# kan-bayashi/espnet

Hardware: AMD Instinct MI355X
Metric: frames/sec, 12L Conformer hybrid CTC/attention training step (B=32 T=1000 d=256 per GPU) (higher is better)
Workload: dtype f32; 1 GPU; BASELINE configs[1]: 12L Conformer enc d=256 h=4 ff=2048 k=31 macaron+cnn rel_pos, 6L Transformer dec, V=5000, fbank B=32 T=1000 L=100, mtlalpha 0.3, lsm 0.1; global_batch=32, frames=1000, parallelism=dp1, optimizer=adam+noam, clip 5.0, launch=hipGraph, wgrad_side_stream=False, optimizer_steps_done=114

## Files before the change

### espnet_amd/csrc/attn_f32.hip

```cpp
#include "common.h"

namespace {

constexpr int ATT_DK = 64;
constexpr int ATT_MAXK = 512;
constexpr int PLD = 68;

struct AttnF32Args {
  const float* qu; const float* qv; const float* k; const float* v; const float* pos;
  const unsigned char* mask;
  float* P; float* ctx;
  long ldq, ldqv, ldk, ldv, ldpos, ldc, ldp, mb, mi;
  int B, H, T1, T2, nqb;
  float scale;
  float* Pd; float drop_p; const unsigned long long* drop_step; unsigned long long drop_salt;
  const int* tshift;
};

__device__ __forceinline__ float xmax16_32(float v) {
  v = fmaxf(v, __shfl_xor(v, 16));
  return fmaxf(v, __shfl_xor(v, 32));
}
__device__ __forceinline__ float xsum16_32(float v) {
  v += __shfl_xor(v, 16);
  return v + __shfl_xor(v, 32);
}

__device__ __forceinline__ void load_frag(const float* row, int fq, float4 (&f)[4]) {
#pragma unroll
  for (int j = 0; j < 4; ++j) f[j] = *reinterpret_cast<const float4*>(row + 16 * j + 4 * fq);
}
__device__ __forceinline__ f32x4 dot_tile(const float4 (&x)[4], const float4 (&y)[4], f32x4 c) {
#pragma unroll
  for (int j = 0; j < 4; ++j) {
    c = __builtin_amdgcn_mfma_f32_16x16x4f32(x[j].x, y[j].x, c, 0, 0, 0);
    c = __builtin_amdgcn_mfma_f32_16x16x4f32(x[j].y, y[j].y, c, 0, 0, 0);
    c = __builtin_amdgcn_mfma_f32_16x16x4f32(x[j].z, y[j].z, c, 0, 0, 0);
    c = __builtin_amdgcn_mfma_f32_16x16x4f32(x[j].w, y[j].w, c, 0, 0, 0);
  }
  return c;
}

template <int NKT>
__device__ __forceinline__ void panel_load(const float* src, long ld, int rows, int t, float4 (&r)[NKT]) {
#pragma unroll
  for (int q = 0; q < NKT; ++q) {
    const int c = t + 256 * q, row = c >> 4, c4 = c & 15;
    r[q] = *reinterpret_cast<const float4*>(src + (long)min(row, rows - 1) * ld + c4 * 4);
    if (row >= rows) r[q] = make_float4(0.f, 0.f, 0.f, 0.f);
  }
}
template <int NKT>
__device__ __forceinline__ void panel_store(const float4 (&r)[NKT], float* dst, int t) {
#pragma unroll
  for (int q = 0; q < NKT; ++q) {
    const int c = t + 256 * q, row = c >> 4, c4 = c & 15;
    *reinterpret_cast<float4*>(&dst[row * PLD + c4 * 4]) = r[q];
  }
}

template <int NKT>
__device__ __forceinline__ void panel_product(const float* panel, const f32x4 (&G)[NKT], int fr, int fq, f32x4 (&C)[4]) {
#pragma unroll
  for (int kt = 0; kt < NKT; ++kt)
#pragma unroll
    for (int r = 0; r < 4; ++r) {
      const float* row = &panel[(kt * 16 + 4 * fq + r) * PLD + fr];
#pragma unroll
      for (int dt = 0; dt < 4; ++dt) C[dt] = __builtin_amdgcn_mfma_f32_16x16x4f32(row[dt * 16], G[kt][r], C[dt], 0, 0, 0);
    }
}

template <int NKT, bool ACC>
__device__ __forceinline__ void score_tiles(const float* keys, long ldk, int T2, const float* qs, long ldq, int nq,
                                            float* X, int XLD, int wave, int fr, int fq) {
  constexpr int TPW = NKT / 4;
  float4 qf[4][4];
#pragma unroll
  for (int qt = 0; qt < 4; ++qt) load_frag(qs + (long)min(qt * 16 + fr, nq - 1) * ldq, fq, qf[qt]);
#pragma unroll
  for (int u = 0; u < TPW; ++u) {
    const int kt = wave * TPW + u;
    float4 kf[4];
    load_frag(keys + (long)min(kt * 16 + fr, T2 - 1) * ldk, fq, kf);
#pragma unroll
    for (int qt = 0; qt < 4; ++qt) {
      f32x4 c = (f32x4){0.f, 0.f, 0.f, 0.f};
      float4* xp = reinterpret_cast<float4*>(&X[(qt * 16 + fr) * XLD + kt * 16 + 4 * fq]);
      if (ACC) {
        const float4 o = *xp;
        c = (f32x4){o.x, o.y, o.z, o.w};
      }
      c = dot_tile(kf, qf[qt], c);
      *xp = make_float4(c[0], c[1], c[2], c[3]);
    }
  }
}

template <bool REL, int NKT>
__global__ __launch_bounds__(256, NKT > 16 ? 1 : 2) void attn_f32_fwd_kernel(const AttnF32Args a) {
  extern __shared__ __attribute__((aligned(16))) char smem_raw[];
  constexpr int XLD = NKT * 16 + 4;
  constexpr int TPW = NKT / 4;
  const int t = threadIdx.x, lane = t & 63, wave = t >> 6;
  const int fr = lane & 15, fq = lane >> 4;
  const int xcd = blockIdx.x & 7, jb = blockIdx.x >> 3;
  const int z = (jb / a.nqb) * 8 + xcd;
  const bool live = z < a.B * a.H;
  const int zz = live ? z : 0;
  const int h = zz / a.B, b = zz % a.B;
  const int T1 = a.T1, T2 = a.T2;
  const int r0w = min((jb % a.nqb) * 64, T1 - 1);
  const int nq = T1 - r0w;
  const int r0 = r0w + wave * 16;
  const bool active = live && r0 < T1;
  const int qi = min(r0 + fr, T1 - 1);

  float* X = reinterpret_cast<float*>(smem_raw);
  const int Ts = (REL && a.tshift) ? min(max(a.tshift[0], 1), T2) : T2;
  if (REL) {
    if (Ts < T2) {
      for (int e = t; e < 64 * XLD; e += 256) X[e] = 0.f;
      __syncthreads();
    }
    float4 qf[4][4];
    const float* qs = a.qv + ((long)b * T1 + r0w) * a.ldqv + h * ATT_DK;
#pragma unroll
    for (int qt = 0; qt < 4; ++qt) load_frag(qs + (long)min(qt * 16 + fr, nq - 1) * a.ldqv, fq, qf[qt]);
    if (t < 64 && r0w + t + 1 < T2) X[t * XLD + r0w + t + 1] = 0.f;
#pragma unroll
    for (int u = 0; u < TPW; ++u) {
      const int mt = wave * TPW + u;
      float4 pf[4];
      load_frag(a.pos + (long)min(mt * 16 + fr, T2 - 1) * a.ldpos + h * ATT_DK, fq, pf);
#pragma unroll
      for (int qt = 0; qt < 4; ++qt) {
        const f32x4 c = dot_tile(pf, qf[qt], (f32x4){0.f, 0.f, 0.f, 0.f});
        const int ql = qt * 16 + fr, i = r0w + ql;
        const int lim = Ts - 1 - i;
#pragma unroll
        for (int r = 0; r < 4; ++r) {
          const int m = mt * 16 + 4 * fq + r;
          const int row = m >= lim ? ql : ql - 1, j = m >= lim ? m - lim : m + i + 1;
          if (m < Ts && i < Ts && ql < nq && row >= 0) X[row * XLD + j] = c[r];
        }
      }
    }
    const int i64 = r0w + 64;
    if (live && i64 < Ts) {
      const float4* qr = reinterpret_cast<const float4*>(a.qv + ((long)b * T1 + i64) * a.ldqv + h * ATT_DK);
      for (int m = t; m <= Ts - 2 - i64; m += 256) {
        const float4* pr = reinterpret_cast<const float4*>(a.pos + (long)m * a.ldpos + h * ATT_DK);
        float s = 0.f;
#pragma unroll
        for (int j = 0; j < 16; ++j) {
          const float4 x = qr[j], y = pr[j];
          s += x.x * y.x + x.y * y.y + x.z * y.z + x.w * y.w;
        }
        X[63 * XLD + m + i64 + 1] = s;
      }
    }
    __syncthreads();
  }
  score_tiles<NKT, REL>(a.k + (long)b * T2 * a.ldk + h * ATT_DK, a.ldk, T2, a.qu + ((long)b * T1 + r0w) * a.ldq + h * ATT_DK,
                        a.ldq, nq, X, XLD, wave, fr, fq);
  float4 vreg[NKT];
  panel_load<NKT>(a.v + (long)b * T2 * a.ldv + h * ATT_DK, a.ldv, live ? T2 : 1, t, vreg);
  __syncthreads();
  f32x4 S[NKT];
  if (active) {
    unsigned mk[NKT];
    if (a.mask) {
      const unsigned char* mr = a.mask + (long)b * a.mb + (long)qi * a.mi;
#pragma unroll
      for (int kt = 0; kt < NKT; ++kt) {
        const int j0 = kt * 16 + fq * 4;
        const unsigned m0 = mr[min(j0, T2 - 1)], m1 = mr[min(j0 + 1, T2 - 1)], m2 = mr[min(j0 + 2, T2 - 1)],
                       m3 = mr[min(j0 + 3, T2 - 1)];
        mk[kt] = m0 | (m1 << 8) | (m2 << 16) | (m3 << 24);
      }
    } else {
#pragma unroll
      for (int kt = 0; kt < NKT; ++kt) mk[kt] = 0x01010101u;
    }
    const float* xrow = &X[(wave * 16 + fr) * XLD + 4 * fq];
    float mx = -INFINITY;
#pragma unroll
    for (int kt = 0; kt < NKT; ++kt) {
      const int j0 = kt * 16 + fq * 4;
      const float4 xv = *reinterpret_cast<const float4*>(xrow + kt * 16);
      const float xs[4] = {xv.x, xv.y, xv.z, xv.w};
#pragma unroll
      for (int r = 0; r < 4; ++r) {
        float x = xs[r] * a.scale;
        if (j0 + r >= T2 || ((mk[kt] >> (8 * r)) & 0xffu) == 0u) x = -INFINITY;
        S[kt][r] = x;
        mx = fmaxf(mx, x);
      }
    }
    mx = xmax16_32(mx);
    const bool dead = mx == -INFINITY;
    float sum = 0.f;
#pragma unroll
    for (int kt = 0; kt < NKT; ++kt)
#pragma unroll
      for (int r = 0; r < 4; ++r) {
        const float e = dead ? 0.f : __expf(S[kt][r] - mx);
        S[kt][r] = e;
        sum += e;
      }
    sum = xsum16_32(sum);
    const float inv = dead ? 0.f : 1.f / sum;
    const bool qok = r0 + fr < T1;
    const long pro = ((long)zz * T1 + qi) * a.ldp;
    float* prow = a.P + pro;
#pragma unroll
    for (int kt = 0; kt < NKT; ++kt) {
      S[kt] *= inv;
      const int j0 = kt * 16 + fq * 4;
      if (qok && j0 < a.ldp)
        *reinterpret_cast<float4*>(prow + j0) = make_float4(S[kt][0], S[kt][1], S[kt][2], S[kt][3]);
    }
    if (a.drop_p > 0.f) {
      const unsigned seed = eamd_drop_seed(a.drop_step, a.drop_salt), thr = eamd_drop_thr16(a.drop_p);
      const float dinv = eamd_drop_inv(thr);
#pragma unroll
      for (int kt = 0; kt < NKT; ++kt) {
        const int j0 = kt * 16 + fq * 4;
        bool kp[4];
        eamd_drop_keep4(seed, (unsigned long long)(pro + min(j0, (int)a.ldp - 4)), thr, kp);
#pragma unroll
        for (int r = 0; r < 4; ++r) S[kt][r] = kp[r] ? S[kt][r] * dinv : 0.f;
        if (qok && j0 < a.ldp)
          *reinterpret_cast<float4*>(a.Pd + pro + j0) = make_float4(S[kt][0], S[kt][1], S[kt][2], S[kt][3]);
      }
    }
  } else {
#pragma unroll
    for (int kt = 0; kt < NKT; ++kt) S[kt] = (f32x4){0.f, 0.f, 0.f, 0.f};
  }
  __syncthreads();
  float* Vs = reinterpret_cast<float*>(smem_raw);
  panel_store<NKT>(vreg, Vs, t);
  __syncthreads();
  if (!active) return;
  f32x4 C[4];
#pragma unroll
  for (int dt = 0; dt < 4; ++dt) C[dt] = (f32x4){0.f, 0.f, 0.f, 0.f};
  panel_product<NKT>(Vs, S, fr, fq, C);
  if (r0 + fr < T1) {
    float* crow = a.ctx + ((long)b * T1 + r0 + fr) * a.ldc + h * ATT_DK;
#pragma unroll
    for (int dt = 0; dt < 4; ++dt)
      *reinterpret_cast<float4*>(crow + dt * 16 + fq * 4) = make_float4(C[dt][0], C[dt][1], C[dt][2], C[dt][3]);
  }
}

struct AttnF32BwdArgs {
  const float* dctx; const float* k; const float* v; const float* P;
  float* dS; float* dbd; float* dq;
  long ldd, ldk, ldv, ldp, ldo;
  int B, H, T1, T2, nqb;
  float scale;
  float drop_p; const unsigned long long* drop_step; unsigned long long drop_salt;
  const int* tshift;
};

template <int NKT>
__global__ __launch_bounds__(256, NKT > 16 ? 1 : 2) void attn_f32_bwd_q_kernel(const AttnF32BwdArgs a) {
  extern __shared__ __attribute__((aligned(16))) char smem_raw[];
  constexpr int XLD = NKT * 16 + 4;
  const int t = threadIdx.x, lane = t & 63, wave = t >> 6;
  const int fr = lane & 15, fq = lane >> 4;
  const int xcd = blockIdx.x & 7, jb = blockIdx.x >> 3;
  const int z = (jb / a.nqb) * 8 + xcd;
  const bool live = z < a.B * a.H;
  const int zz = live ? z : 0;
  const int h = zz / a.B, b = zz % a.B;
  const int T1 = a.T1, T2 = a.T2;
  const int Ts = (a.dbd && a.tshift) ? min(max(a.tshift[0], 1), T2) : T2;
  const int r0w = min((jb % a.nqb) * 64, T1 - 1);
  const int nq = T1 - r0w;
  const int r0 = r0w + wave * 16;
  const bool active = live && r0 < T1;
  const int qi = min(r0 + fr, T1 - 1);
  const bool qok = r0 + fr < T1;

  float* X = reinterpret_cast<float*>(smem_raw);
  score_tiles<NKT, false>(a.v + (long)b * T2 * a.ldv + h * ATT_DK, a.ldv, T2,
                          a.dctx + ((long)b * T1 + r0w) * a.ldd + h * ATT_DK, a.ldd, nq, X, XLD, wave, fr, fq);
  const float* prow = a.P + ((long)zz * T1 + qi) * a.ldp;
  float4 Pr[NKT];
#pragma unroll
  for (int kt = 0; kt < NKT; ++kt) {
    const int j0 = kt * 16 + fq * 4;
    Pr[kt] = *reinterpret_cast<const float4*>(prow + min(j0, (int)a.ldp - 4));
    if (j0 >= (int)a.ldp) Pr[kt] = make_float4(0.f, 0.f, 0.f, 0.f);
  }
  __syncthreads();
  f32x4 S[NKT];
  if (active) {
    const float* xrow = &X[(wave * 16 + fr) * XLD + 4 * fq];
    const bool drop = a.drop_p > 0.f;
    const unsigned seed = drop ? eamd_drop_seed(a.drop_step, a.drop_salt) : 0u, thr = eamd_drop_thr16(a.drop_p);
    const float dinv = eamd_drop_inv(thr);
    const long pro = ((long)zz * T1 + qi) * a.ldp;
    float s = 0.f;
#pragma unroll
    for (int kt = 0; kt < NKT; ++kt) {
      const int j0 = kt * 16 + fq * 4;
      const float4 xv = *reinterpret_cast<const float4*>(xrow + kt * 16);
      S[kt] = (f32x4){xv.x, xv.y, xv.z, xv.w};
      if (drop) {
        bool kp[4];
        eamd_drop_keep4(seed, (unsigned long long)(pro + min(j0, (int)a.ldp - 4)), thr, kp);
#pragma unroll
        for (int r = 0; r < 4; ++r) S[kt][r] = kp[r] ? S[kt][r] * dinv : 0.f;
      }
      const float pr[4] = {Pr[kt].x, Pr[kt].y, Pr[kt].z, Pr[kt].w};
#pragma unroll
      for (int r = 0; r < 4; ++r) if (j0 + r < T2) s += pr[r] * S[kt][r];
    }
    s = xsum16_32(s);
    const long zo = (long)zz * T1 * a.ldp;
    float* srow = a.dS + zo + (long)qi * a.ldp;
    const int i = r0 + fr;
#pragma unroll
    for (int kt = 0; kt < NKT; ++kt) {
      const int j0 = kt * 16 + fq * 4;
      const float pr[4] = {Pr[kt].x, Pr[kt].y, Pr[kt].z, Pr[kt].w};
#pragma unroll
      for (int r = 0; r < 4; ++r) {
        const int j = j0 + r;
        const float g = j < T2 ? pr[r] * (S[kt][r] - s) * a.scale : 0.f;
        S[kt][r] = g;
        if (a.dbd && qok) {
          if (j < Ts && i < Ts) {
            const int R = j <= i ? i : i + 1, c = j <= i ? Ts + j - i : j - i - 1;
            if (c != 0) a.dbd[zo + (long)R * a.ldp + (c - 1)] = g;
          } else if (j < (int)a.ldp) {
            a.dbd[zo + (long)i * a.ldp + j] = 0.f;
          }
        }
      }
      if (qok && j0 < (int)a.ldp) *reinterpret_cast<float4*>(srow + j0) = make_float4(S[kt][0], S[kt][1], S[kt][2], S[kt][3]);
    }
    if (a.dbd && r0 == 0)
      for (int f = 1 + lane; f < Ts; f += 64) a.dbd[zo + (f - 1)] = 0.f;
  } else {
#pragma unroll
    for (int kt = 0; kt < NKT; ++kt) S[kt] = (f32x4){0.f, 0.f, 0.f, 0.f};
  }
  float4 kreg[NKT];
  panel_load<NKT>(a.k + (long)b * T2 * a.ldk + h * ATT_DK, a.ldk, live ? T2 : 1, t, kreg);
  __syncthreads();
  float* Ks = reinterpret_cast<float*>(smem_raw);
  panel_store<NKT>(kreg, Ks, t);
  __syncthreads();
  if (!active) return;
  f32x4 C[4];
#pragma unroll
  for (int dt = 0; dt < 4; ++dt) C[dt] = (f32x4){0.f, 0.f, 0.f, 0.f};
  panel_product<NKT>(Ks, S, fr, fq, C);
  if (qok) {
    float* orow = a.dq + ((long)b * T1 + r0 + fr) * a.ldo + h * ATT_DK;
#pragma unroll
    for (int dt = 0; dt < 4; ++dt)
      *reinterpret_cast<float4*>(orow + dt * 16 + fq * 4) = make_float4(C[dt][0], C[dt][1], C[dt][2], C[dt][3]);
  }
}

constexpr int ATT_LONG_MAXK = 4096;

typedef unsigned short bfbits;
__device__ __forceinline__ float bf2f_(unsigned short b) { return __uint_as_float((unsigned)b << 16); }
__device__ __forceinline__ float4 ld4(const float* p) { return *reinterpret_cast<const float4*>(p); }
__device__ __forceinline__ float4 ld4(const bfbits* p) {
  const uint2 u = *reinterpret_cast<const uint2*>(p);
  return make_float4(bf2f_(u.x & 0xffffu), bf2f_(u.x >> 16), bf2f_(u.y & 0xffffu), bf2f_(u.y >> 16));
}
__device__ __forceinline__ void st4(float* p, float4 v) { *reinterpret_cast<float4*>(p) = v; }
__device__ __forceinline__ void st4(bfbits* p, float4 v) {
  uint2 u;
  u.x = (unsigned)eamd_f2bf(v.x) | ((unsigned)eamd_f2bf(v.y) << 16);
  u.y = (unsigned)eamd_f2bf(v.z) | ((unsigned)eamd_f2bf(v.w) << 16);
  *reinterpret_cast<uint2*>(p) = u;
}
__device__ __forceinline__ void st1(float* p, float v) { *p = v; }
__device__ __forceinline__ void st1(bfbits* p, float v) { *p = eamd_f2bf(v); }
__device__ __forceinline__ float rnd(const float*, float v) { return v; }
__device__ __forceinline__ float rnd(const bfbits*, float v) { return bf2f_(eamd_f2bf(v)); }
template <typename T>
__device__ __forceinline__ void load_frag_t(const T* row, int fq, float4 (&f)[4]) {
#pragma unroll
  for (int j = 0; j < 4; ++j) f[j] = ld4(row + 16 * j + 4 * fq);
}

template <typename T>
__device__ __forceinline__ void tile_load(const T* src, long ld, int key0, int T2, int lane, float4 (&r)[4]) {
#pragma unroll
  for (int q = 0; q < 4; ++q) {
    const int c = lane + 64 * q, row = c >> 4, c4 = c & 15;
    r[q] = ld4(src + (long)min(key0 + row, T2 - 1) * ld + c4 * 4);
    if (key0 + row >= T2) r[q] = make_float4(0.f, 0.f, 0.f, 0.f);
  }
}
__device__ __forceinline__ void tile_store(const float4 (&r)[4], float* dst, int lane) {
#pragma unroll
  for (int q = 0; q < 4; ++q) {
    const int c = lane + 64 * q, row = c >> 4, c4 = c & 15;
    *reinterpret_cast<float4*>(&dst[row * PLD + c4 * 4]) = r[q];
  }
}
__device__ __forceinline__ void tile_product(const float* tile, const f32x4& G, int fr, int fq, f32x4 (&C)[4]) {
#pragma unroll
  for (int r = 0; r < 4; ++r) {
    const float* row = &tile[(4 * fq + r) * PLD + fr];
#pragma unroll
    for (int dt = 0; dt < 4; ++dt) C[dt] = __builtin_amdgcn_mfma_f32_16x16x4f32(row[dt * 16], G[r], C[dt], 0, 0, 0);
  }
}
template <int NW, typename T>
__device__ __forceinline__ void reduce_store_ct(const f32x4 (&C)[4], float* scr, int wave, int fr, int fq, int t, T* out,
                                                long ld, int nq) {
#pragma unroll
  for (int dt = 0; dt < 4; ++dt)
#pragma unroll
    for (int r = 0; r < 4; ++r) scr[(wave * 64 + dt * 16 + fq * 4 + r) * 17 + fr] = C[dt][r];
  __syncthreads();
  const int q = t >> 4, c4 = (t & 15) * 4;
  if (q < nq) {
    float o[4];
#pragma unroll
    for (int e = 0; e < 4; ++e) {
      float v = 0.f;
#pragma unroll
      for (int w = 0; w < NW; ++w) v += scr[(w * 64 + c4 + e) * 17 + q];
      o[e] = v;
    }
    st4(out + (long)q * ld + c4, make_float4(o[0], o[1], o[2], o[3]));
  }
}

template <typename T, bool REL, int LQ, int NW>
__global__ __launch_bounds__(64 * NW) void attn_fwd_long_kernel(const AttnF32Args a, const int nkt) {
  constexpr int QT = LQ >= 16 ? LQ / 16 : 1;
  constexpr int NT = 64 * NW;
  const T* const a_qu = reinterpret_cast<const T*>(a.qu); const T* const a_qv = reinterpret_cast<const T*>(a.qv);
  const T* const a_k = reinterpret_cast<const T*>(a.k); const T* const a_v = reinterpret_cast<const T*>(a.v);
  const T* const a_pos = reinterpret_cast<const T*>(a.pos);
  T* const a_P = reinterpret_cast<T*>(a.P); T* const a_Pd = reinterpret_cast<T*>(a.Pd); T* const a_ctx = reinterpret_cast<T*>(a.ctx);
  extern __shared__ __attribute__((aligned(16))) char smem_raw[];
  const int XLD = nkt * 16 + 4;
  const int t = threadIdx.x, lane = t & 63, wave = t >> 6;
  const int fr = lane & 15, fq = lane >> 4;
  const int xcd = blockIdx.x & 7, jb = blockIdx.x >> 3;
  const int z = (jb / a.nqb) * 8 + xcd;
  const bool live = z < a.B * a.H;
  const int zz = live ? z : 0;
  const int h = zz / a.B, b = zz % a.B;
  const int T1 = a.T1, T2 = a.T2;
  const int r0w = min((jb % a.nqb) * LQ, T1 - 1);
  const int nq = min(LQ, T1 - r0w);
  int rowx[QT], qrow[QT], qi[QT];
  bool qok[QT];
#pragma unroll
  for (int qt = 0; qt < QT; ++qt) {
    rowx[qt] = min(fr + 16 * qt, LQ - 1);
    qrow[qt] = r0w + min(fr + 16 * qt, nq - 1);
    qi[qt] = min(r0w + rowx[qt], T1 - 1);
    qok[qt] = live && fr + 16 * qt < nq;
  }
  float* X = reinterpret_cast<float*>(smem_raw);
  float* Tw = X + LQ * XLD + wave * 16 * PLD;
  float* red = X + LQ * XLD + NW * 16 * PLD;
  const int Ts = (REL && a.tshift) ? min(max(a.tshift[0], 1), T2) : T2;
  if (REL) {
    if (Ts < T2) {
      for (int e = t; e < LQ * XLD; e += NT) X[e] = 0.f;
      __syncthreads();
    }
    float4 qf[QT][4];
#pragma unroll
    for (int qt = 0; qt < QT; ++qt) load_frag_t(a_qv + ((long)b * T1 + qrow[qt]) * a.ldqv + h * ATT_DK, fq, qf[qt]);
    if (t < LQ && r0w + t + 1 < T2) X[t * XLD + r0w + t + 1] = 0.f;
    float4 pf[4], pfn[4];
    if (wave < nkt) load_frag_t(a_pos + (long)min(wave * 16 + fr, T2 - 1) * a.ldpos + h * ATT_DK, fq, pf);
    for (int mt = wave; mt < nkt; mt += NW) {
      if (mt + NW < nkt) load_frag_t(a_pos + (long)min((mt + NW) * 16 + fr, T2 - 1) * a.ldpos + h * ATT_DK, fq, pfn);
#pragma unroll
      for (int qt = 0; qt < QT; ++qt) {
        const f32x4 c = dot_tile(pf, qf[qt], (f32x4){0.f, 0.f, 0.f, 0.f});
        const int lr = fr + 16 * qt;
        const int i = r0w + lr, lim = Ts - 1 - i;
#pragma unroll
        for (int r = 0; r < 4; ++r) {
          const int m = mt * 16 + 4 * fq + r;
          const int row = m >= lim ? lr : lr - 1, j = m >= lim ? m - lim : m + i + 1;
          if (m < Ts && i < Ts && lr < nq && row >= 0) X[row * XLD + j] = c[r];
        }
      }
#pragma unroll
// ... 172 lines not shown
    qok[qt] = live && fr + 16 * qt < nq;
  }
  float* X = reinterpret_cast<float*>(smem_raw);
  float* Tw = X + LQ * XLD + wave * 16 * PLD;
  float* red = X + LQ * XLD + NW * 16 * PLD;
  const bool drop = a.drop_p > 0.f;
  const unsigned seed = drop ? eamd_drop_seed(a.drop_step, a.drop_salt) : 0u, thr = eamd_drop_thr16(a.drop_p);
  const float dinv = eamd_drop_inv(thr);
  float s[QT];
  {
    float4 df[QT][4];
#pragma unroll
    for (int qt = 0; qt < QT; ++qt) {
      s[qt] = 0.f;
      load_frag_t(a_dctx + ((long)b * T1 + qrow[qt]) * a.ldd + h * ATT_DK, fq, df[qt]);
    }
    const T* vs = a_v + (long)b * T2 * a.ldv + h * ATT_DK;
    float4 vf[4], vfn[4];
    if (wave < nkt) load_frag_t(vs + (long)min(wave * 16 + fr, T2 - 1) * a.ldv, fq, vf);
    for (int kt = wave; kt < nkt; kt += NW) {
      if (kt + NW < nkt) load_frag_t(vs + (long)min((kt + NW) * 16 + fr, T2 - 1) * a.ldv, fq, vfn);
      const int j0 = kt * 16 + fq * 4;
#pragma unroll
      for (int qt = 0; qt < QT; ++qt) {
        f32x4 c = dot_tile(vf, df[qt], (f32x4){0.f, 0.f, 0.f, 0.f});
        float4 pr = ld4(a_P + pro[qt] + min(j0, (int)a.ldp - 4));
        if (j0 >= (int)a.ldp) pr = make_float4(0.f, 0.f, 0.f, 0.f);
        if (drop) {
          bool kp[4];
          eamd_drop_keep4(seed, (unsigned long long)(pro[qt] + min(j0, (int)a.ldp - 4)), thr, kp);
#pragma unroll
          for (int r = 0; r < 4; ++r) c[r] = kp[r] ? c[r] * dinv : 0.f;
        }
        const float p4[4] = {pr.x, pr.y, pr.z, pr.w};
#pragma unroll
        for (int r = 0; r < 4; ++r) if (j0 + r < T2) s[qt] += p4[r] * c[r];
        *reinterpret_cast<float4*>(&X[rowx[qt] * XLD + kt * 16 + 4 * fq]) = make_float4(c[0], c[1], c[2], c[3]);
      }
#pragma unroll
      for (int j = 0; j < 4; ++j) vf[j] = vfn[j];
    }
  }
#pragma unroll
  for (int qt = 0; qt < QT; ++qt) {
    s[qt] = xsum16_32(s[qt]);
    if (fq == 0) red[wave * LQ + rowx[qt]] = s[qt];
  }
  __syncthreads();
#pragma unroll
  for (int qt = 0; qt < QT; ++qt) {
    const int rx = rowx[qt];
    float s_ = 0.f;
#pragma unroll
    for (int w_ = 0; w_ < NW; w_ += 2) s_ += red[w_ * LQ + rx] + red[(w_ + 1) * LQ + rx];
    s[qt] = s_;
  }
  const T* ks = a_k + (long)b * T2 * a.ldk + h * ATT_DK;
  f32x4 C[QT][4];
#pragma unroll
  for (int qt = 0; qt < QT; ++qt)
#pragma unroll
    for (int dt = 0; dt < 4; ++dt) C[qt][dt] = (f32x4){0.f, 0.f, 0.f, 0.f};
  float4 kreg[4];
  if (wave < nkt) tile_load(ks, a.ldk, wave * 16, live ? T2 : 1, lane, kreg);
  for (int kt = wave; kt < nkt; kt += NW) {
    tile_store(kreg, Tw, lane);
    if (kt + NW < nkt) tile_load(ks, a.ldk, (kt + NW) * 16, live ? T2 : 1, lane, kreg);
    const int j0 = kt * 16 + fq * 4;
#pragma unroll
    for (int qt = 0; qt < QT; ++qt) {
      const int i = r0w + fr + 16 * qt;
      float4 pr = ld4(a_P + pro[qt] + min(j0, (int)a.ldp - 4));
      if (j0 >= (int)a.ldp) pr = make_float4(0.f, 0.f, 0.f, 0.f);
      const float4 dp = *reinterpret_cast<const float4*>(&X[rowx[qt] * XLD + kt * 16 + 4 * fq]);
      const float p4[4] = {pr.x, pr.y, pr.z, pr.w}, d4[4] = {dp.x, dp.y, dp.z, dp.w};
      f32x4 G;
#pragma unroll
      for (int r = 0; r < 4; ++r) {
        const int j = j0 + r;
        const float g = j < T2 ? p4[r] * (d4[r] - s[qt]) * a.scale : 0.f;
        G[r] = g;
        if (a.dbd && qok[qt]) {
          if (j < Ts && i < Ts) {
            const int R = j <= i ? i : i + 1, c = j <= i ? Ts + j - i : j - i - 1;
            if (c != 0) st1(a_dbd + zo + (long)R * a.ldp + (c - 1), g);
          } else if (j < (int)a.ldp) {
            st1(a_dbd + zo + (long)i * a.ldp + j, 0.f);
          }
        }
      }
      if (qok[qt] && j0 < (int)a.ldp) st4(a_dS + pro[qt] + j0, make_float4(G[0], G[1], G[2], G[3]));
#pragma unroll
      for (int r = 0; r < 4; ++r) G[r] = rnd(a_dS, G[r]);
      tile_product(Tw, G, fr, fq, C[qt]);
    }
  }
  if (a.dbd && live && r0w == 0)
    for (int f = 1 + t; f < Ts; f += NT) st1(a_dbd + zo + (f - 1), 0.f);
  __syncthreads();
#pragma unroll
  for (int qt = 0; qt < QT; ++qt) {
    if (qt > 0) __syncthreads();
    const int nqt = live ? max(0, min(16, nq - 16 * qt)) : 0;
    const long orow = ((long)b * T1 + r0w + 16 * qt) * a.ldo + h * ATT_DK;
    if (dq_bf16)
      reduce_store_ct<NW>(C[qt], X, wave, fr, fq, t, reinterpret_cast<bfbits*>(a.dq) + orow, a.ldo, nqt);
    else
      reduce_store_ct<NW>(C[qt], X, wave, fr, fq, t, a.dq + orow, a.ldo, nqt);
  }
}

template <typename T, bool REL, int LQ, int NW>
int launch_fwd_long_q(AttnF32Args a, hipStream_t stream) {
  const int nkt = (a.T2 + 15) / 16;
  const size_t smem = ((size_t)LQ * (nkt * 16 + 4) + NW * 16 * PLD + 2 * NW * LQ) * sizeof(float);
  if (smem > 160 * 1024 || smem < (size_t)NW * 64 * 17 * sizeof(float)) return EAMD_EUNSUPPORTED;
  static const hipError_t attr_err = hipFuncSetAttribute(reinterpret_cast<const void*>(&attn_fwd_long_kernel<T, REL, LQ, NW>),
                                                         hipFuncAttributeMaxDynamicSharedMemorySize, 160 * 1024);
  if (attr_err != hipSuccess) return (int)attr_err;
  a.nqb = (a.T1 + LQ - 1) / LQ;
  const int nz = (a.B * a.H + 7) / 8 * 8;
  if ((long)a.nqb * nz >= (1L << 31)) return EAMD_EUNSUPPORTED;
  hipLaunchKernelGGL((attn_fwd_long_kernel<T, REL, LQ, NW>), dim3((unsigned)(a.nqb * nz)), dim3(64 * NW), smem, stream, a, nkt);
  EAMD_LAUNCH_CHECK();
  return EAMD_OK;
}
struct LongGeom { int lq, nw; };
inline LongGeom long_geom(int T1, int T2) {
  const int nkt = (T2 + 15) / 16;
  auto bytes = [&](int lq, int nw) { return ((size_t)lq * (nkt * 16 + 4) + nw * 16 * PLD + 2 * nw * lq) * sizeof(float); };
  LongGeom g{16, 4};
  if (bytes(16, 4) > 160 * 1024) g = LongGeom{8, 4};
  if (bytes(g.lq, 4) > 80 * 1024) g.nw = bytes(g.lq, 8) <= 160 * 1024 ? 8 : bytes(g.lq, 6) <= 160 * 1024 ? 6 : 4;
  (void)T1;
  return g;
}
template <typename T, bool REL>
int launch_fwd_long(AttnF32Args a, hipStream_t stream) {
  const LongGeom g = long_geom(a.T1, a.T2);
  if (g.lq == 16) return g.nw == 8 ? launch_fwd_long_q<T, REL, 16, 8>(a, stream) : g.nw == 6 ? launch_fwd_long_q<T, REL, 16, 6>(a, stream)
                                                                                               : launch_fwd_long_q<T, REL, 16, 4>(a, stream);
  return g.nw == 8 ? launch_fwd_long_q<T, REL, 8, 8>(a, stream) : g.nw == 6 ? launch_fwd_long_q<T, REL, 8, 6>(a, stream)
                                                                              : launch_fwd_long_q<T, REL, 8, 4>(a, stream);
}

template <typename T, int LQ, int NW>
int launch_bwd_long_q(AttnF32BwdArgs a, int dq_bf16, hipStream_t stream) {
  const int nkt = (a.T2 + 15) / 16;
  const size_t smem = ((size_t)LQ * (nkt * 16 + 4) + NW * 16 * PLD + 2 * NW * LQ) * sizeof(float);
  if (smem > 160 * 1024 || smem < (size_t)NW * 64 * 17 * sizeof(float)) return EAMD_EUNSUPPORTED;
  static const hipError_t attr_err = hipFuncSetAttribute(reinterpret_cast<const void*>(&attn_bwd_q_long_kernel<T, LQ, NW>),
                                                         hipFuncAttributeMaxDynamicSharedMemorySize, 160 * 1024);
  if (attr_err != hipSuccess) return (int)attr_err;
  a.nqb = (a.T1 + LQ - 1) / LQ;
  const int nz = (a.B * a.H + 7) / 8 * 8;
  if ((long)a.nqb * nz >= (1L << 31)) return EAMD_EUNSUPPORTED;
  hipLaunchKernelGGL((attn_bwd_q_long_kernel<T, LQ, NW>), dim3((unsigned)(a.nqb * nz)), dim3(64 * NW), smem, stream, a, nkt, dq_bf16);
  EAMD_LAUNCH_CHECK();
  return EAMD_OK;
}
template <typename T>
int launch_bwd_long(AttnF32BwdArgs a, int dq_bf16, hipStream_t stream) {
  const LongGeom g = long_geom(a.T1, a.T2);
  if (g.lq == 16) return g.nw == 8 ? launch_bwd_long_q<T, 16, 8>(a, dq_bf16, stream) : launch_bwd_long_q<T, 16, 4>(a, dq_bf16, stream);
  return g.nw == 8 ? launch_bwd_long_q<T, 8, 8>(a, dq_bf16, stream) : launch_bwd_long_q<T, 8, 4>(a, dq_bf16, stream);
}

template <bool REL, int NKT>
int launch_fwd(const AttnF32Args& a, size_t smem, hipStream_t stream) {
  static const hipError_t attr_err = hipFuncSetAttribute(reinterpret_cast<const void*>(&attn_f32_fwd_kernel<REL, NKT>),
                                                         hipFuncAttributeMaxDynamicSharedMemorySize, NKT * 16 * PLD * 4);
  if (attr_err != hipSuccess) return (int)attr_err;
  const int nz = (a.B * a.H + 7) / 8 * 8;
  hipLaunchKernelGGL((attn_f32_fwd_kernel<REL, NKT>), dim3((unsigned)(a.nqb * nz)), dim3(256), smem, stream, a);
  EAMD_LAUNCH_CHECK();
  return EAMD_OK;
}

template <int NKT>
int launch_bwd(const AttnF32BwdArgs& a, hipStream_t stream) {
  static const hipError_t attr_err = hipFuncSetAttribute(reinterpret_cast<const void*>(&attn_f32_bwd_q_kernel<NKT>),
                                                         hipFuncAttributeMaxDynamicSharedMemorySize, NKT * 16 * PLD * 4);
  if (attr_err != hipSuccess) return (int)attr_err;
  const int nz = (a.B * a.H + 7) / 8 * 8;
  hipLaunchKernelGGL((attn_f32_bwd_q_kernel<NKT>), dim3((unsigned)(a.nqb * nz)), dim3(256),
                     (size_t)NKT * 16 * PLD * sizeof(float), stream, a);
  EAMD_LAUNCH_CHECK();
  return EAMD_OK;
}

bool al16(const void* p) { return (reinterpret_cast<uintptr_t>(p) & 15) == 0; }

}

int eamd_attn_long_fwd_bf16(const void* qu, int64_t ldq, const void* qv, int64_t ldqv, const void* k, int64_t ldk, const void* v,
                            int64_t ldv, const void* pos, int64_t ldpos, const unsigned char* mask, int64_t mb, int64_t mi,
                            void* P, int64_t ldp, void* ctx, int64_t ldc, int B, int H, int T1, int T2, float scale, void* Pd,
                            float drop_p, const uint64_t* drop_step, uint64_t drop_salt, const int32_t* shift_len, void* stream) {
  if (T2 > ATT_LONG_MAXK || ldq % 4 || ldk % 4 || ldv % 4 || ldc % 4 || ldp % 4) return EAMD_EUNSUPPORTED;
  AttnF32Args a;
  a.qu = (const float*)qu; a.qv = (const float*)qv; a.k = (const float*)k; a.v = (const float*)v; a.pos = (const float*)pos;
  a.mask = mask; a.P = (float*)P; a.ctx = (float*)ctx;
  a.ldq = ldq; a.ldqv = ldqv; a.ldk = ldk; a.ldv = ldv; a.ldpos = ldpos; a.ldc = ldc; a.ldp = ldp; a.mb = mb; a.mi = mi;
  a.B = B; a.H = H; a.T1 = T1; a.T2 = T2; a.nqb = 0; a.scale = scale;
  a.Pd = (float*)Pd; a.drop_p = drop_p; a.drop_step = (const unsigned long long*)drop_step; a.drop_salt = drop_salt;
  a.tshift = shift_len;
  return pos ? launch_fwd_long<bfbits, true>(a, (hipStream_t)stream) : launch_fwd_long<bfbits, false>(a, (hipStream_t)stream);
}

int eamd_attn_long_bwd_q_bf16(const void* dctx, int64_t ldd, const void* k, int64_t ldk, const void* v, int64_t ldv, const void* P,
                              int64_t ldp, void* dS, void* dbd, void* dq, int64_t ldo, int dq_is_bf16, int B, int H, int T1, int T2,
                              float scale, float drop_p, const uint64_t* drop_step, uint64_t drop_salt, const int32_t* shift_len,
                              void* stream) {
  if (T2 > ATT_LONG_MAXK || ldd % 4 || ldk % 4 || ldv % 4 || ldp % 4 || ldo % 4) return EAMD_EUNSUPPORTED;
  AttnF32BwdArgs a;
  a.dctx = (const float*)dctx; a.k = (const float*)k; a.v = (const float*)v; a.P = (const float*)P;
  a.dS = (float*)dS; a.dbd = (float*)dbd; a.dq = (float*)dq;
  a.ldd = ldd; a.ldk = ldk; a.ldv = ldv; a.ldp = ldp; a.ldo = ldo;
  a.B = B; a.H = H; a.T1 = T1; a.T2 = T2; a.nqb = 0; a.scale = scale;
  a.drop_p = drop_p; a.drop_step = (const unsigned long long*)drop_step; a.drop_salt = drop_salt;
  a.tshift = shift_len;
  return launch_bwd_long<bfbits>(a, dq_is_bf16, (hipStream_t)stream);
}

extern "C" int eamd_attn_fwd_f32(const float* qu, int64_t ldq, const float* qv, int64_t ldqv, const float* k, int64_t ldk,
                                 const float* v, int64_t ldv, const float* pos, int64_t ldpos, const unsigned char* mask,
                                 int64_t mask_bstride, int64_t mask_qstride, float* P, int64_t ldp, float* ctx,
                                 int64_t ldc, int B, int H, int T1, int T2, int dk, float scale, float* Pd, float drop_p,
                                 const uint64_t* drop_step, uint64_t drop_salt, const int32_t* shift_len, void* stream) {
  if (!qu || !k || !v || !P || !ctx || B <= 0 || H <= 0 || T1 <= 0 || T2 <= 0) return EAMD_EINVAL;
  if (drop_p < 0.f || drop_p >= 1.f || (drop_p > 0.f && (!Pd || !drop_step || !al16(Pd)))) return EAMD_EINVAL;
  if ((pos == nullptr) != (qv == nullptr)) return EAMD_EINVAL;
  if (dk != ATT_DK || T2 > ATT_LONG_MAXK || (pos && T1 != T2)) return EAMD_EUNSUPPORTED;
  if (ldq % 4 || ldk % 4 || ldv % 4 || ldc % 4 || ldp % 4 || ldp < T2 || (pos && (ldqv % 4 || ldpos % 4)))
    return EAMD_EUNSUPPORTED;
  if (!al16(qu) || !al16(k) || !al16(v) || !al16(P) || !al16(ctx) || (pos && (!al16(qv) || !al16(pos))))
    return EAMD_EUNSUPPORTED;
  if ((long)B * H * ((T1 + 63) / 64) >= (1L << 28)) return EAMD_EUNSUPPORTED;
  AttnF32Args a;
  a.qu = qu; a.qv = qv; a.k = k; a.v = v; a.pos = pos; a.mask = mask; a.P = P; a.ctx = ctx;
  a.ldq = ldq; a.ldqv = ldqv; a.ldk = ldk; a.ldv = ldv; a.ldpos = ldpos; a.ldc = ldc; a.ldp = ldp;
  a.mb = mask_bstride; a.mi = mask_qstride;
  a.B = B; a.H = H; a.T1 = T1; a.T2 = T2; a.nqb = (T1 + 63) / 64; a.scale = scale;
  a.Pd = Pd; a.drop_p = drop_p; a.drop_step = (const unsigned long long*)drop_step; a.drop_salt = drop_salt;
  a.tshift = shift_len;
  if (T2 > ATT_MAXK) return pos ? launch_fwd_long<float, true>(a, (hipStream_t)stream) : launch_fwd_long<float, false>(a, (hipStream_t)stream);
  const int nkt = T2 <= 128 ? 8 : T2 <= 256 ? 16 : 32;
  const size_t smem = (size_t)nkt * 16 * PLD * sizeof(float);
  hipStream_t s = (hipStream_t)stream;
  if (pos) return nkt == 8 ? launch_fwd<true, 8>(a, smem, s) : nkt == 16 ? launch_fwd<true, 16>(a, smem, s) : launch_fwd<true, 32>(a, smem, s);
  return nkt == 8 ? launch_fwd<false, 8>(a, smem, s) : nkt == 16 ? launch_fwd<false, 16>(a, smem, s) : launch_fwd<false, 32>(a, smem, s);
}

extern "C" int eamd_attn_bwd_q_f32(const float* dctx, int64_t ldd, const float* k, int64_t ldk, const float* v, int64_t ldv,
                                   const float* P, int64_t ldp, float* dS, float* dbd, float* dq, int64_t ldo, int B, int H,
                                   int T1, int T2, int dk, float scale, float drop_p, const uint64_t* drop_step,
                                   uint64_t drop_salt, const int32_t* shift_len, void* stream) {
  if (!dctx || !k || !v || !P || !dS || !dq || B <= 0 || H <= 0 || T1 <= 0 || T2 <= 0) return EAMD_EINVAL;
  if (drop_p < 0.f || drop_p >= 1.f || (drop_p > 0.f && !drop_step)) return EAMD_EINVAL;
  if (dk != ATT_DK || T2 > ATT_LONG_MAXK || (dbd && T1 != T2)) return EAMD_EUNSUPPORTED;
  if (ldd % 4 || ldk % 4 || ldv % 4 || ldp % 4 || ldp < T2 || ldo % 4) return EAMD_EUNSUPPORTED;
  if (!al16(dctx) || !al16(k) || !al16(v) || !al16(P) || !al16(dS) || !al16(dq)) return EAMD_EUNSUPPORTED;
  if ((long)B * H * ((T1 + 63) / 64) >= (1L << 28)) return EAMD_EUNSUPPORTED;
  AttnF32BwdArgs a;
  a.dctx = dctx; a.k = k; a.v = v; a.P = P; a.dS = dS; a.dbd = dbd; a.dq = dq;
  a.ldd = ldd; a.ldk = ldk; a.ldv = ldv; a.ldp = ldp; a.ldo = ldo;
  a.B = B; a.H = H; a.T1 = T1; a.T2 = T2; a.nqb = (T1 + 63) / 64; a.scale = scale;
  a.drop_p = drop_p; a.drop_step = (const unsigned long long*)drop_step; a.drop_salt = drop_salt;
  a.tshift = shift_len;
  if (T2 > ATT_MAXK) return launch_bwd_long<float>(a, 0, (hipStream_t)stream);
  return T2 <= 128 ? launch_bwd<8>(a, (hipStream_t)stream) : T2 <= 256 ? launch_bwd<16>(a, (hipStream_t)stream)
                                                                         : launch_bwd<32>(a, (hipStream_t)stream);
}

namespace {

constexpr int KLD = 80;

struct AttnF32KvArgs {
  const float* Pd; const float* dS; const float* dbd;
  const float* dctx; const float* qu; const float* qv;
  float* dv; float* dk; float* dpos;
  long ldp, ldd, ldq, ldqv, ldo, ldpos;
  int B, H, T1, T2, nkb;
};

__device__ __forceinline__ void kv_tile_load(const float* src, long ld, int i0, int T1, int c0, int ncol, int t, float4 (&r)[4]) {
#pragma unroll
  for (int q = 0; q < 4; ++q) {
    const int c = t + 256 * q, row = c >> 4, c4 = c & 15;
    const bool ok = i0 + row < T1 && c0 + c4 * 4 < ncol;
    r[q] = *reinterpret_cast<const float4*>(src + (long)min(i0 + row, T1 - 1) * ld + (ok ? c0 + c4 * 4 : 0));
    if (!ok) r[q] = make_float4(0.f, 0.f, 0.f, 0.f);
  }
}
__device__ __forceinline__ void kv_tile_store(const float4 (&r)[4], float* dst, int t) {
#pragma unroll
  for (int q = 0; q < 4; ++q) {
    const int c = t + 256 * q, row = c >> 4, c4 = c & 15;
    *reinterpret_cast<float4*>(&dst[row * KLD + c4 * 4]) = r[q];
  }
}
__device__ __forceinline__ void kv_product(const float* Xc, const float* Wk, int wave, int fr, int fq, f32x4 (&acc)[4]) {
#pragma unroll
  for (int kk = 0; kk < 16; ++kk) {
    const int i = 4 * kk + fq;
    const float b = Wk[i * KLD + wave * 16 + fr];
#pragma unroll
    for (int ct = 0; ct < 4; ++ct)
      acc[ct] = __builtin_amdgcn_mfma_f32_16x16x4f32(Xc[i * KLD + ct * 16 + fr], b, acc[ct], 0, 0, 0);
  }
}

template <bool REL>
__global__ __launch_bounds__(256, 2) void attn_f32_bwd_kv_kernel(const AttnF32KvArgs a) {
  __shared__ __attribute__((aligned(16))) float sW[64 * KLD];
  __shared__ __attribute__((aligned(16))) float sX[64 * KLD];
  const int t = threadIdx.x, lane = t & 63, wave = t >> 6;
  const int fr = lane & 15, fq = lane >> 4;
  const int xcd = blockIdx.x & 7, jb = blockIdx.x >> 3;
  const int z = (jb / a.nkb) * 8 + xcd;
  if (z >= a.B * a.H) return;
  const int h = z / a.B, b = z % a.B;
  const int T1 = a.T1, T2 = a.T2;
  const int j0 = (jb % a.nkb) * 64;
  const long zo = (long)z * T1 * a.ldp;
  const float* Wsrc[3] = {a.Pd + zo, a.dS + zo, REL ? a.dbd + zo : nullptr};
  const float* Xsrc[3] = {a.dctx + (long)b * T1 * a.ldd + h * ATT_DK, a.qu + (long)b * T1 * a.ldq + h * ATT_DK,
                          REL ? a.qv + (long)b * T1 * a.ldqv + h * ATT_DK : nullptr};
  const long Xld[3] = {a.ldd, a.ldq, a.ldqv};
  constexpr int NP = REL ? 3 : 2;
  f32x4 acc[NP][4];
#pragma unroll
  for (int p = 0; p < NP; ++p)
#pragma unroll
    for (int ct = 0; ct < 4; ++ct) acc[p][ct] = (f32x4){0.f, 0.f, 0.f, 0.f};
  const int nstage = ((T1 + 63) / 64) * NP;
  float4 rw[4], rx[4];
  kv_tile_load(Wsrc[0], a.ldp, 0, T1, j0, (int)a.ldp, t, rw);
  kv_tile_load(Xsrc[0], Xld[0], 0, T1, 0, 64, t, rx);
  for (int s = 0; s < nstage; ++s) {
    const int p = s % NP;
    __syncthreads();
    kv_tile_store(rw, sW, t);
    kv_tile_store(rx, sX, t);
    __syncthreads();
    if (s + 1 < nstage) {
      const int pn = (s + 1) % NP, i0 = (s + 1) / NP * 64;
      if (pn == 0) { kv_tile_load(Wsrc[0], a.ldp, i0, T1, j0, (int)a.ldp, t, rw); kv_tile_load(Xsrc[0], Xld[0], i0, T1, 0, 64, t, rx); }
      else if (pn == 1) { kv_tile_load(Wsrc[1], a.ldp, i0, T1, j0, (int)a.ldp, t, rw); kv_tile_load(Xsrc[1], Xld[1], i0, T1, 0, 64, t, rx); }
      else if (REL) { kv_tile_load(Wsrc[2], a.ldp, i0, T1, j0, (int)a.ldp, t, rw); kv_tile_load(Xsrc[2], Xld[2], i0, T1, 0, 64, t, rx); }
    }
    if (p == 0) kv_product(sX, sW, wave, fr, fq, acc[0]);
    else if (p == 1) kv_product(sX, sW, wave, fr, fq, acc[1]);
    else if (REL) kv_product(sX, sW, wave, fr, fq, acc[NP - 1]);
  }
  const int j = j0 + wave * 16 + fr;
  if (j < T2) {
    float* vrow = a.dv + ((long)b * T2 + j) * a.ldo + h * ATT_DK + 4 * fq;
    float* krow = a.dk + ((long)b * T2 + j) * a.ldo + h * ATT_DK + 4 * fq;
#pragma unroll
    for (int ct = 0; ct < 4; ++ct) {
      *reinterpret_cast<float4*>(vrow + ct * 16) = make_float4(acc[0][ct][0], acc[0][ct][1], acc[0][ct][2], acc[0][ct][3]);
      *reinterpret_cast<float4*>(krow + ct * 16) = make_float4(acc[1][ct][0], acc[1][ct][1], acc[1][ct][2], acc[1][ct][3]);
    }
    if (REL) {
      float* prow = a.dpos + (long)j * a.ldpos + h * ATT_DK + 4 * fq;
#pragma unroll
      for (int ct = 0; ct < 4; ++ct)
#pragma unroll
        for (int r = 0; r < 4; ++r) atomicAdd(prow + ct * 16 + r, acc[NP - 1][ct][r]);
    }
  }
}

}

extern "C" int eamd_attn_bwd_kv_f32(const float* Pd, const float* dS, const float* dbd, int64_t ldp, const float* dctx,
                                    int64_t ldd, const float* qu, int64_t ldq, const float* qv, int64_t ldqv, float* dv,
                                    float* dk_out, int64_t ldo, float* dpos, int64_t ldpos, int B, int H, int T1, int T2, int dk,
                                    void* stream) {
  if (!Pd || !dS || !dctx || !qu || !dv || !dk_out || B <= 0 || H <= 0 || T1 <= 0 || T2 <= 0) return EAMD_EINVAL;
  if ((dbd == nullptr) != (qv == nullptr) || (dbd == nullptr) != (dpos == nullptr)) return EAMD_EINVAL;
  if (dk != ATT_DK || (dbd && T1 != T2)) return EAMD_EUNSUPPORTED;
  if (ldp % 4 || ldp < T2 || ldd % 4 || ldq % 4 || ldo % 4 || (dbd && (ldqv % 4 || ldpos % 4))) return EAMD_EUNSUPPORTED;
  if (!al16(Pd) || !al16(dS) || !al16(dctx) || !al16(qu) || !al16(dv) || !al16(dk_out) ||
      (dbd && (!al16(dbd) || !al16(qv) || !al16(dpos))))
    return EAMD_EUNSUPPORTED;
  AttnF32KvArgs a;
  a.Pd = Pd; a.dS = dS; a.dbd = dbd; a.dctx = dctx; a.qu = qu; a.qv = qv; a.dv = dv; a.dk = dk_out; a.dpos = dpos;
  a.ldp = ldp; a.ldd = ldd; a.ldq = ldq; a.ldqv = ldqv; a.ldo = ldo; a.ldpos = ldpos;
  a.B = B; a.H = H; a.T1 = T1; a.T2 = T2; a.nkb = (T2 + 63) / 64;
  if ((long)B * H * a.nkb >= (1L << 28)) return EAMD_EUNSUPPORTED;
  const int nz = (B * H + 7) / 8 * 8;
  hipStream_t s = (hipStream_t)stream;
  if (dbd) hipLaunchKernelGGL((attn_f32_bwd_kv_kernel<true>), dim3((unsigned)(a.nkb * nz)), dim3(256), 0, s, a);
  else hipLaunchKernelGGL((attn_f32_bwd_kv_kernel<false>), dim3((unsigned)(a.nkb * nz)), dim3(256), 0, s, a);
  EAMD_LAUNCH_CHECK();
  return EAMD_OK;
}
```

Measured before the change: 1.125 million frames/s.

## Software-pipeline attention score and KV-grad kernels with prefetch and double buffering

In the forward attention kernel, key and position fragments are now prefetched one tile ahead, and the four query tiles are interleaved in the MFMA chain. The mask is also precomputed into a keep bitmask before the score phase, and the relative-position scatter uses a branchless store into a padding column. In the KV backward kernel, the shared tiles are double-buffered in dynamic shared memory, which removes one barrier per stage, and the LDS operand reads are register-prefetched. The aim is to hide global and LDS load latency behind MFMA work, at the cost of more registers and doubled LDS that could lower occupancy.

```diff
diff --git a/espnet_amd/csrc/attn_f32.hip b/espnet_amd/csrc/attn_f32.hip
--- a/espnet_amd/csrc/attn_f32.hip
+++ b/espnet_amd/csrc/attn_f32.hip
@@ -40,6 +40,19 @@
   }
   return c;
 }
+__device__ __forceinline__ void dot_tiles4(const float4 (&x)[4], const float4 (&y)[4][4], f32x4 (&c)[4]) {
+#pragma unroll
+  for (int j = 0; j < 4; ++j) {
+#pragma unroll
+    for (int qt = 0; qt < 4; ++qt) c[qt] = __builtin_amdgcn_mfma_f32_16x16x4f32(x[j].x, y[qt][j].x, c[qt], 0, 0, 0);
+#pragma unroll
+    for (int qt = 0; qt < 4; ++qt) c[qt] = __builtin_amdgcn_mfma_f32_16x16x4f32(x[j].y, y[qt][j].y, c[qt], 0, 0, 0);
+#pragma unroll
+    for (int qt = 0; qt < 4; ++qt) c[qt] = __builtin_amdgcn_mfma_f32_16x16x4f32(x[j].z, y[qt][j].z, c[qt], 0, 0, 0);
+#pragma unroll
+    for (int qt = 0; qt < 4; ++qt) c[qt] = __builtin_amdgcn_mfma_f32_16x16x4f32(x[j].w, y[qt][j].w, c[qt], 0, 0, 0);
+  }
+}
 
 template <int NKT>
 __device__ __forceinline__ void panel_load(const float* src, long ld, int rows, int t, float4 (&r)[NKT]) {
@@ -75,25 +88,29 @@
 __device__ __forceinline__ void score_tiles(const float* keys, long ldk, int T2, const float* qs, long ldq, int nq,
                                             float* X, int XLD, int wave, int fr, int fq) {
   constexpr int TPW = NKT / 4;
-  float4 qf[4][4];
+  float4 qf[4][4], kf[4], kfn[4];
+  load_frag(keys + (long)min(wave * TPW * 16 + fr, T2 - 1) * ldk, fq, kf);
 #pragma unroll
   for (int qt = 0; qt < 4; ++qt) load_frag(qs + (long)min(qt * 16 + fr, nq - 1) * ldq, fq, qf[qt]);
 #pragma unroll
   for (int u = 0; u < TPW; ++u) {
     const int kt = wave * TPW + u;
-    float4 kf[4];
-    load_frag(keys + (long)min(kt * 16 + fr, T2 - 1) * ldk, fq, kf);
+    if (u + 1 < TPW) load_frag(keys + (long)min((kt + 1) * 16 + fr, T2 - 1) * ldk, fq, kfn);
+    f32x4 c[4];
 #pragma unroll
     for (int qt = 0; qt < 4; ++qt) {
-      f32x4 c = (f32x4){0.f, 0.f, 0.f, 0.f};
-      float4* xp = reinterpret_cast<float4*>(&X[(qt * 16 + fr) * XLD + kt * 16 + 4 * fq]);
+      c[qt] = (f32x4){0.f, 0.f, 0.f, 0.f};
       if (ACC) {
-        const float4 o = *xp;
-        c = (f32x4){o.x, o.y, o.z, o.w};
-      }
-      c = dot_tile(kf, qf[qt], c);
-      *xp = make_float4(c[0], c[1], c[2], c[3]);
-    }
+        const float4 o = *reinterpret_cast<const float4*>(&X[(qt * 16 + fr) * XLD + kt * 16 + 4 * fq]);
+        c[qt] = (f32x4){o.x, o.y, o.z, o.w};
+      }
+    }
+    dot_tiles4(kf, qf, c);
+#pragma unroll
+    for (int qt = 0; qt < 4; ++qt)
+      *reinterpret_cast<float4*>(&X[(qt * 16 + fr) * XLD + kt * 16 + 4 * fq]) = make_float4(c[qt][0], c[qt][1], c[qt][2], c[qt][3]);
+#pragma unroll
+    for (int j = 0; j < 4; ++j) kf[j] = kfn[j];
   }
 }
 
@@ -117,34 +134,61 @@
   const int qi = min(r0 + fr, T1 - 1);
 
   float* X = reinterpret_cast<float*>(smem_raw);
+  unsigned keep[NKT / 8];
+#pragma unroll
+  for (int w = 0; w < NKT / 8; ++w) keep[w] = 0u;
+  if (a.mask) {
+    const unsigned char* mr = a.mask + (long)b * a.mb + (long)qi * a.mi;
+    unsigned mbyte[NKT][4];
+#pragma unroll
+    for (int kt = 0; kt < NKT; ++kt)
+#pragma unroll
+      for (int r = 0; r < 4; ++r) mbyte[kt][r] = mr[min(kt * 16 + fq * 4 + r, T2 - 1)];
+#pragma unroll
+    for (int kt = 0; kt < NKT; ++kt)
+#pragma unroll
+      for (int r = 0; r < 4; ++r)
+        keep[kt / 8] |= (unsigned)((mbyte[kt][r] != 0u) & (kt * 16 + fq * 4 + r < T2)) << (4 * (kt % 8) + r);
+  } else {
+#pragma unroll
+    for (int kt = 0; kt < NKT; ++kt)
+#pragma unroll
+      for (int r = 0; r < 4; ++r) keep[kt / 8] |= (unsigned)(kt * 16 + fq * 4 + r < T2) << (4 * (kt % 8) + r);
+  }
   const int Ts = (REL && a.tshift) ? min(max(a.tshift[0], 1), T2) : T2;
   if (REL) {
     if (Ts < T2) {
       for (int e = t; e < 64 * XLD; e += 256) X[e] = 0.f;
       __syncthreads();
     }
-    float4 qf[4][4];
+    float4 qf[4][4], pf[4], pfn[4];
     const float* qs = a.qv + ((long)b * T1 + r0w) * a.ldqv + h * ATT_DK;
+    load_frag(a.pos + (long)min(wave * TPW * 16 + fr, T2 - 1) * a.ldpos + h * ATT_DK, fq, pf);
 #pragma unroll
     for (int qt = 0; qt < 4; ++qt) load_frag(qs + (long)min(qt * 16 + fr, nq - 1) * a.ldqv, fq, qf[qt]);
     if (t < 64 && r0w + t + 1 < T2) X[t * XLD + r0w + t + 1] = 0.f;
 #pragma unroll
     for (int u = 0; u < TPW; ++u) {
       const int mt = wave * TPW + u;
-      float4 pf[4];
-      load_frag(a.pos + (long)min(mt * 16 + fr, T2 - 1) * a.ldpos + h * ATT_DK, fq, pf);
+      if (u + 1 < TPW) load_frag(a.pos + (long)min((mt + 1) * 16 + fr, T2 - 1) * a.ldpos + h * ATT_DK, fq, pfn);
+      f32x4 c[4];
+#pragma unroll
+      for (int qt = 0; qt < 4; ++qt) c[qt] = (f32x4){0.f, 0.f, 0.f, 0.f};
+      dot_tiles4(pf, qf, c);
 #pragma unroll
       for (int qt = 0; qt < 4; ++qt) {
-        const f32x4 c = dot_tile(pf, qf[qt], (f32x4){0.f, 0.f, 0.f, 0.f});
         const int ql = qt * 16 + fr, i = r0w + ql;
         const int lim = Ts - 1 - i;
 #pragma unroll
         for (int r = 0; r < 4; ++r) {
           const int m = mt * 16 + 4 * fq + r;
           const int row = m >= lim ? ql : ql - 1, j = m >= lim ? m - lim : m + i + 1;
-          if (m < Ts && i < Ts && ql < nq && row >= 0) X[row * XLD + j] = c[r];
+          const bool st = m < Ts && i < Ts && ql < nq && row >= 0;
+          X[st ? row * XLD + j : ql * XLD + NKT * 16 + fq] = c[qt][r];
         }
       }
+#pragma unroll
+      for (int j = 0; j < 4; ++j) pf[j] = pfn[j];
     }
     const int i64 = r0w + 64;
     if (live && i64 < Ts) {
@@ -169,35 +213,21 @@
   __syncthreads();
   f32x4 S[NKT];
   if (active) {
-    unsigned mk[NKT];
-    if (a.mask) {
-      const unsigned char* mr = a.mask + (long)b * a.mb + (long)qi * a.mi;
-#pragma unroll
-      for (int kt = 0; kt < NKT; ++kt) {
-        const int j0 = kt * 16 + fq * 4;
-        const unsigned m0 = mr[min(j0, T2 - 1)], m1 = mr[min(j0 + 1, T2 - 1)], m2 = mr[min(j0 + 2, T2 - 1)],
-                       m3 = mr[min(j0 + 3, T2 - 1)];
-        mk[kt] = m0 | (m1 << 8) | (m2 << 16) | (m3 << 24);
-      }
-    } else {
-#pragma unroll
-      for (int kt = 0; kt < NKT; ++kt) mk[kt] = 0x01010101u;
-    }
     const float* xrow = &X[(wave * 16 + fr) * XLD + 4 * fq];
+#pragma unroll
+    for (int kt = 0; kt < NKT; ++kt) {
+      const float4 xv = *reinterpret_cast<const float4*>(xrow + kt * 16);
+      S[kt] = (f32x4){xv.x, xv.y, xv.z, xv.w};
+    }
     float mx = -INFINITY;
 #pragma unroll
-    for (int kt = 0; kt < NKT; ++kt) {
-      const int j0 = kt * 16 + fq * 4;
-      const float4 xv = *reinterpret_cast<const float4*>(xrow + kt * 16);
-      const float xs[4] = {xv.x, xv.y, xv.z, xv.w};
+    for (int kt = 0; kt < NKT; ++kt)
 #pragma unroll
       for (int r = 0; r < 4; ++r) {
-        float x = xs[r] * a.scale;
-        if (j0 + r >= T2 || ((mk[kt] >> (8 * r)) & 0xffu) == 0u) x = -INFINITY;
+        const float x = ((keep[kt / 8] >> (4 * (kt % 8) + r)) & 1u) ? S[kt][r] * a.scale : -INFINITY;
         S[kt][r] = x;
         mx = fmaxf(mx, x);
       }
-    }
     mx = xmax16_32(mx);
     const bool dead = mx == -INFINITY;
     float sum = 0.f;
@@ -976,20 +1006,34 @@
   }
 }
 __device__ __forceinline__ void kv_product(const float* Xc, const float* Wk, int wave, int fr, int fq, f32x4 (&acc)[4]) {
-#pragma unroll
-  for (int kk = 0; kk < 16; ++kk) {
-    const int i = 4 * kk + fq;
-    const float b = Wk[i * KLD + wave * 16 + fr];
-#pragma unroll
-    for (int ct = 0; ct < 4; ++ct)
-      acc[ct] = __builtin_amdgcn_mfma_f32_16x16x4f32(Xc[i * KLD + ct * 16 + fr], b, acc[ct], 0, 0, 0);
-  }
-}
+  float bw[2][4], xc[2][4][4];
+  auto fetch = [&](int g, float (&b_)[4], float (&x_)[4][4]) {
+#pragma unroll
+    for (int u = 0; u < 4; ++u) {
+      const int i = 4 * (4 * g + u) + fq;
+      b_[u] = Wk[i * KLD + wave * 16 + fr];
+#pragma unroll
+      for (int ct = 0; ct < 4; ++ct) x_[u][ct] = Xc[i * KLD + ct * 16 + fr];
+    }
+  };
+  fetch(0, bw[0], xc[0]);
+#pragma unroll
+  for (int g = 0; g < 4; ++g) {
+    if (g + 1 < 4) fetch(g + 1, bw[(g + 1) & 1], xc[(g + 1) & 1]);
+#pragma unroll
+    for (int u = 0; u < 4; ++u)
+#pragma unroll
+      for (int ct = 0; ct < 4; ++ct)
+        acc[ct] = __builtin_amdgcn_mfma_f32_16x16x4f32(xc[g & 1][u][ct], bw[g & 1][u], acc[ct], 0, 0, 0);
+  }
+}
+
+constexpr size_t KV_SMEM = 2 * 2 * 64 * KLD * sizeof(float);
 
 template <bool REL>
 __global__ __launch_bounds__(256, 2) void attn_f32_bwd_kv_kernel(const AttnF32KvArgs a) {
-  __shared__ __attribute__((aligned(16))) float sW[64 * KLD];
-  __shared__ __attribute__((aligned(16))) float sX[64 * KLD];
+  extern __shared__ __attribute__((aligned(16))) char smem_raw[];
+  float* const sbuf = reinterpret_cast<float*>(smem_raw);
   const int t = threadIdx.x, lane = t & 63, wave = t >> 6;
   const int fr = lane & 15, fq = lane >> 4;
   const int xcd = blockIdx.x & 7, jb = blockIdx.x >> 3;
@@ -1013,21 +1057,27 @@
   float4 rw[4], rx[4];
   kv_tile_load(Wsrc[0], a.ldp, 0, T1, j0, (int)a.ldp, t, rw);
   kv_tile_load(Xsrc[0], Xld[0], 0, T1, 0, 64, t, rx);
+  kv_tile_store(rw, sbuf, t);
+  kv_tile_store(rx, sbuf + 64 * KLD, t);
+  __syncthreads();
   for (int s = 0; s < nstage; ++s) {
     const int p = s % NP;
-    __syncthreads();
-    kv_tile_store(rw, sW, t);
-    kv_tile_store(rx, sX, t);
-    __syncthreads();
+    float* const sW = sbuf + (s & 1) * 2 * 64 * KLD;
+    float* const sWn = sbuf + ((s + 1) & 1) * 2 * 64 * KLD;
     if (s + 1 < nstage) {
       const int pn = (s + 1) % NP, i0 = (s + 1) / NP * 64;
       if (pn == 0) { kv_tile_load(Wsrc[0], a.ldp, i0, T1, j0, (int)a.ldp, t, rw); kv_tile_load(Xsrc[0], Xld[0], i0, T1, 0, 64, t, rx); }
       else if (pn == 1) { kv_tile_load(Wsrc[1], a.ldp, i0, T1, j0, (int)a.ldp, t, rw); kv_tile_load(Xsrc[1], Xld[1], i0, T1, 0, 64, t, rx); }
       else if (REL) { kv_tile_load(Wsrc[2], a.ldp, i0, T1, j0, (int)a.ldp, t, rw); kv_tile_load(Xsrc[2], Xld[2], i0, T1, 0, 64, t, rx); }
     }
-    if (p == 0) kv_product(sX, sW, wave, fr, fq, acc[0]);
-    else if (p == 1) kv_product(sX, sW, wave, fr, fq, acc[1]);
-    else if (REL) kv_product(sX, sW, wave, fr, fq, acc[NP - 1]);
+    if (p == 0) kv_product(sW + 64 * KLD, sW, wave, fr, fq, acc[0]);
+    else if (p == 1) kv_product(sW + 64 * KLD, sW, wave, fr, fq, acc[1]);
+    else if (REL) kv_product(sW + 64 * KLD, sW, wave, fr, fq, acc[NP - 1]);
+    if (s + 1 < nstage) {
+      kv_tile_store(rw, sWn, t);
+      kv_tile_store(rx, sWn + 64 * KLD, t);
+    }
+    __syncthreads();
   }
   const int j = j0 + wave * 16 + fr;
   if (j < T2) {
@@ -1068,8 +1118,12 @@
   if ((long)B * H * a.nkb >= (1L << 28)) return EAMD_EUNSUPPORTED;
   const int nz = (B * H + 7) / 8 * 8;
   hipStream_t s = (hipStream_t)stream;
-  if (dbd) hipLaunchKernelGGL((attn_f32_bwd_kv_kernel<true>), dim3((unsigned)(a.nkb * nz)), dim3(256), 0, s, a);
-  else hipLaunchKernelGGL((attn_f32_bwd_kv_kernel<false>), dim3((unsigned)(a.nkb * nz)), dim3(256), 0, s, a);
+  static const hipError_t attr_err[2] = {
+      hipFuncSetAttribute(reinterpret_cast<const void*>(&attn_f32_bwd_kv_kernel<false>), hipFuncAttributeMaxDynamicSharedMemorySize, KV_SMEM),
+      hipFuncSetAttribute(reinterpret_cast<const void*>(&attn_f32_bwd_kv_kernel<true>), hipFuncAttributeMaxDynamicSharedMemorySize, KV_SMEM)};
+  if (attr_err[dbd ? 1 : 0] != hipSuccess) return (int)attr_err[dbd ? 1 : 0];
+  if (dbd) hipLaunchKernelGGL((attn_f32_bwd_kv_kernel<true>), dim3((unsigned)(a.nkb * nz)), dim3(256), KV_SMEM, s, a);
+  else hipLaunchKernelGGL((attn_f32_bwd_kv_kernel<false>), dim3((unsigned)(a.nkb * nz)), dim3(256), KV_SMEM, s, a);
   EAMD_LAUNCH_CHECK();
   return EAMD_OK;
 }
```

Measured after the change: 1.128 million frames/s, median of 6. Within noise of the previous version (+0.3%).
